# MarkJhonBao/InfantPoseEstimation_GaussianBias

Measured on AMD Instinct MI355X. Metric: images/sec (train fwd+bwd) HRFormer-S 256x192, higher is better.
Workload: dtype bf16; 1 GPU; HRFormer-small + fusion head, 256x192 -> 64x48, K=17, train step fwd+bwd+AdamW, DropPath 0.1, BN train; global_batch=64, per_gpu_batch=64, parallelism=dp1, launch=hipGraph replay, branches on concurrent HIP streams

## Files before the change

infantposeestimation_gaussianbias_amd/csrc/pk_block.hip:

```cpp
#include "pk_common.h"

typedef __attribute__((ext_vector_type(8))) short bf16x8;
typedef __attribute__((ext_vector_type(4))) float f32x4;
typedef __attribute__((ext_vector_type(4))) short s16x4;
typedef __attribute__((ext_vector_type(4))) unsigned int u32x4;
typedef __attribute__((ext_vector_type(2))) unsigned int u32x2;

#define OOB_OFF 0x80000000u
#define MAKE_RSRC(ptr) __builtin_amdgcn_make_buffer_rsrc(const_cast<uint16_t*>(ptr), 0, 0x7ffffff0, 0x00020000)
#define LOG2E_F 1.44269504088896340736f
#define MFMA(a, b, c) __builtin_amdgcn_mfma_f32_16x16x32_bf16(a, b, c, 0, 0, 0)
#define MFMA16(a, b, c) __builtin_amdgcn_mfma_f32_16x16x16bf16_1k(a, b, c, 0, 0, 0)
#define LO4(v) __builtin_shufflevector(v, v, 0, 1, 2, 3)
#define HI4(v) __builtin_shufflevector(v, v, 4, 5, 6, 7)
#define LDS_FENCE() asm volatile("s_waitcnt lgkmcnt(0)" ::: "memory")

struct MlpArgs {
    const uint16_t* x;
    const uint16_t* dy;
    uint16_t* out;
    const float *gamma, *beta, *b1, *b2;
    const float* scale;
    const uint16_t* w1;
    const uint16_t* w2;
// ... 302 lines not shown
        for (int s = 0; s < NS; ++s) {
            if (!RESIDENT) {
                __syncthreads();
                if (s + 1 < NS) write_slice((s + 1) & 1);
                if (s + 2 < NS) load_slice(s + 2);
            }
            const u32x4* fr = ring + (RESIDENT ? s : (s & 1)) * NF * 64;
            f32x4 h[RT][2];
#pragma unroll
            for (int u = 0; u < 2; ++u) {
                const f32x4 bias = *reinterpret_cast<const f32x4*>(&sB1[32 * s + 8 * g + 4 * u]);
#pragma unroll
                for (int rt = 0; rt < RT; ++rt) h[rt][u] = bias;
            }
#pragma unroll
            for (int k = 0; k < NK; ++k)
#pragma unroll
                for (int u = 0; u < 2; ++u) {
                    const bf16x8 a = LDS_FRAG(fr, u * NK + k, lane);
#pragma unroll
                    for (int rt = 0; rt < RT; ++rt) h[rt][u] = MFMA(a, vf[rt][k], h[rt][u]);
                }
            bf16x8 hf[RT];
#pragma unroll
            for (int rt = 0; rt < RT; ++rt) {
                hf[rt] = pack2(gelu_erf_poly(h[rt][0]), gelu_erf_poly(h[rt][1]));
            }
#pragma unroll
            for (int ct = 0; ct < NCT; ++ct) {
                const bf16x8 a = LDS_FRAG(fr, 2 * NK + ct, lane);
#pragma unroll
                for (int rt = 0; rt < RT; ++rt) y[rt][ct] = MFMA(a, hf[rt], y[rt][ct]);
            }
        }
#pragma unroll
        for (int rt = 0; rt < RT; ++rt)
#pragma unroll
            for (int ct = 0; ct < NCT; ++ct) {
                const unsigned off = rbase[rt] == OOB_OFF ? OOB_OFF : rbase[rt] + (16 * ct + 4 * g) * 2;
                const u32x2 xo = __builtin_amdgcn_raw_buffer_load_b64(rx, off, 0, 0);
                const f32x4 b2v = __builtin_bit_cast(f32x4, __builtin_amdgcn_raw_buffer_load_b128(rb2, (16 * ct + 4 * g) * 4, 0, 0));
                const f32x4 o = (y[rt][ct] + b2v) * sc[rt] + unpack4(xo);
                __builtin_amdgcn_raw_buffer_store_b64(pack4(o), ro, off, 0, 0);
            }
    };
    if (RESIDENT) {
        for (int grp = blockIdx.x * WAVES + wave; grp < ngroups; grp += gridDim.x * WAVES) process(grp);
    } else {
        process(blockIdx.x * WAVES + wave);
    }
}

template <int C>
__global__ void __launch_bounds__(256) k_mlp_bwd_dx(MlpArgs p) {
    constexpr int HD = 4 * C, NK = C / 32, NT = HD / 16, NS = HD / 32, NCT = C / 16, RT = 2;
    __shared__ __attribute__((aligned(16))) u32x4 sW1[NT * NK * 64];
    __shared__ __attribute__((aligned(16))) u32x4 sW2T[NT * NK * 64];
    __shared__ __attribute__((aligned(16))) u32x4 sW1T[NCT * NS * 64];
    __shared__ __attribute__((aligned(16))) float sB1[HD];
    __shared__ float sRed[4][2][C];
    const int tid = threadIdx.x, lane_ = tid & 63, wave = tid >> 6, i16 = lane_ & 15, g = lane_ >> 4;
    stage_frags(sW1, p.w1, NT * NK, C, [](int f, int i) { return hid(f / NK, i); }, [](int f) { return 32 * (f % NK); });
    stage_frags(sW2T, p.w2t, NT * NK, C, [](int f, int i) { return hid(f / NK, i); }, [](int f) { return 32 * (f % NK); });
    stage_frags(sW1T, p.w1t, NCT * NS, HD, [](int f, int i) { return 16 * (f / NS) + i; }, [](int f) { return 32 * (f % NS); });
    for (int i = tid; i < HD; i += 256) sB1[i] = p.b1[i];
    float gam[NK][8], bet[NK][8];
#pragma unroll
    for (int k = 0; k < NK; ++k)
#pragma unroll
        for (int j = 0; j < 8; ++j) {
            gam[k][j] = p.gamma[32 * k + 8 * g + j];
            bet[k][j] = p.beta[32 * k + 8 * g + j];
        }
    f32x4 gamA[NCT], dgam[NCT], dbet[NCT];
    const f32x4 zero = {0.f, 0.f, 0.f, 0.f};
#pragma unroll
    for (int ct = 0; ct < NCT; ++ct) {
        gamA[ct] = *reinterpret_cast<const f32x4*>(p.gamma + 16 * ct + 4 * g);
        dgam[ct] = dbet[ct] = zero;
    }
    __syncthreads();
    const auto rx = MAKE_RSRC(p.x);
    const auto rg = MAKE_RSRC(p.dy);
    const auto ro = MAKE_RSRC(p.out);
    const int ngroups = (p.M + 16 * RT - 1) / (16 * RT);
    const float inv_c = 1.f / (float)C;
    for (int grp = blockIdx.x * 4 + wave; grp < ngroups; grp += gridDim.x * 4) {
        const int lane = opaque_lane<true>(lane_);
        u32x4 xr[RT][NK], dyr[RT][NK];
        u32x2 xo[RT][NCT], dyo[RT][NCT];
        unsigned rbase[RT];
        float sc[RT];
#pragma unroll
        for (int rt = 0; rt < RT; ++rt) {
            const int row = grp * 16 * RT + 16 * rt + i16;
            const bool ok = row < p.M;
            rbase[rt] = ok ? (unsigned)row * (unsigned)(C * 2) : OOB_OFF;
#pragma unroll
            for (int k = 0; k < NK; ++k) {
                const unsigned off = ok ? rbase[rt] + (32 * k + 8 * g) * 2 : OOB_OFF;
                xr[rt][k] = __builtin_amdgcn_raw_buffer_load_b128(rx, off, 0, 0);
                dyr[rt][k] = __builtin_amdgcn_raw_buffer_load_b128(rg, off, 0, 0);
            }
#pragma unroll
            for (int ct = 0; ct < NCT; ++ct) {
                const unsigned off = ok ? rbase[rt] + (16 * ct + 4 * g) * 2 : OOB_OFF;
                xo[rt][ct] = __builtin_amdgcn_raw_buffer_load_b64(rx, off, 0, 0);
                dyo[rt][ct] = __builtin_amdgcn_raw_buffer_load_b64(rg, off, 0, 0);
            }
            sc[rt] = (p.scale && ok) ? p.scale[row / p.rows_per_sample] : 1.f;
        }
        bf16x8 vf[RT][NK], gf[RT][NK];
        float mean[RT], rstd[RT];
#pragma unroll
        for (int rt = 0; rt < RT; ++rt) {
            ln_row<NK>(xr[rt], gam, bet, inv_c, p.eps, vf[rt], mean[rt], rstd[rt]);
            scale_rows<NK>(dyr[rt], sc[rt], gf[rt]);
        }
        f32x4 dv[RT][NCT];
#pragma unroll
        for (int rt = 0; rt < RT; ++rt)
#pragma unroll
            for (int ct = 0; ct < NCT; ++ct) dv[rt][ct] = zero;
#pragma unroll
        for (int s = 0; s < NS; ++s) {
            f32x4 dz[RT][2];
#pragma unroll
            for (int u = 0; u < 2; ++u) {
                const int t = 2 * s + u;
                const f32x4 bias = *reinterpret_cast<const f32x4*>(&sB1[32 * s + 8 * g + 4 * u]);
                f32x4 z[RT], dh[RT];
#pragma unroll
                for (int rt = 0; rt < RT; ++rt) {
                    z[rt] = bias;
                    dh[rt] = zero;
                }
#pragma unroll
                for (int k = 0; k < NK; ++k) {
                    const bf16x8 a1 = LDS_FRAG(sW1, t * NK + k, lane), a2 = LDS_FRAG(sW2T, t * NK + k, lane);
#pragma unroll
                    for (int rt = 0; rt < RT; ++rt) {
                        z[rt] = MFMA(a1, vf[rt][k], z[rt]);
                        dh[rt] = MFMA(a2, gf[rt][k], dh[rt]);
                    }
                }
#pragma unroll
                for (int rt = 0; rt < RT; ++rt) dz[rt][u] = dh[rt] * gelu_grad(z[rt]);
            }
            bf16x8 dzf[RT];
#pragma unroll
            for (int rt = 0; rt < RT; ++rt) dzf[rt] = pack2(dz[rt][0], dz[rt][1]);
#pragma unroll
            for (int ct = 0; ct < NCT; ++ct) {
                const bf16x8 a = LDS_FRAG(sW1T, ct * NS + s, lane);
#pragma unroll
                for (int rt = 0; rt < RT; ++rt) dv[rt][ct] = MFMA(a, dzf[rt], dv[rt][ct]);
            }
        }
#pragma unroll
        for (int rt = 0; rt < RT; ++rt) {
            f32x4 xh[NCT];
            float s1 = 0.f, s2 = 0.f;
#pragma unroll
            for (int ct = 0; ct < NCT; ++ct) {
                xh[ct] = (unpack4(xo[rt][ct]) - mean[rt]) * rstd[rt];
#pragma unroll
                for (int r = 0; r < 4; ++r) {
                    const float gh = dv[rt][ct][r] * gamA[ct][r];
                    s1 += gh;
                    s2 += gh * xh[ct][r];
                }
                dgam[ct] += dv[rt][ct] * xh[ct];
                dbet[ct] += dv[rt][ct];
            }
            s1 = xor16_sum(s1);
            s1 = xor32_sum(s1);
            s2 = xor16_sum(s2);
            s2 = xor32_sum(s2);
            const float m1 = s1 * inv_c, m2 = s2 * inv_c;
#pragma unroll
            for (int ct = 0; ct < NCT; ++ct) {
                const f32x4 o = (dv[rt][ct] * gamA[ct] - m1 - xh[ct] * m2) * rstd[rt] + unpack4(dyo[rt][ct]);
                __builtin_amdgcn_raw_buffer_store_b64(pack4(o), ro, rbase[rt] == OOB_OFF ? OOB_OFF : rbase[rt] + (16 * ct + 4 * g) * 2, 0, 0);
            }
        }
    }
#pragma unroll
    for (int ct = 0; ct < NCT; ++ct)
#pragma unroll
        for (int r = 0; r < 4; ++r) {
            float a = dgam[ct][r], b = dbet[ct][r];
            a = lanes_sum<16>(a);
            b = lanes_sum<16>(b);
            if (i16 == 0) {
                sRed[wave][0][16 * ct + 4 * g + r] = a;
                sRed[wave][1][16 * ct + 4 * g + r] = b;
            }
        }
    __syncthreads();
    if (tid < 2 * C) {
        const int which = tid / C, c = tid - which * C;
        p.part[(size_t)blockIdx.x * 2 * C + tid] = ((sRed[0][which][c] + sRed[1][which][c]) + sRed[2][which][c]) + sRed[3][which][c];
    }
}

template <int C, int HS>
__global__ void __launch_bounds__(256) k_mlp_bwd_dw(MlpArgs p) {
// ... 928 lines not shown
            f32x4 xh[NCT], gamA[NCT];
            float s1 = 0.f, s2 = 0.f;
#pragma unroll
            for (int ct = 0; ct < NCT; ++ct) {
                gamA[ct] = *reinterpret_cast<const f32x4*>(&sGam[16 * ct + 4 * g]);
                xh[ct] = (unpack4(xo4[t][ct]) - mu) * rsd;
#pragma unroll
                for (int r = 0; r < 4; ++r) {
                    const float gh = du[t][ct][r] * gamA[ct][r];
                    s1 += gh;
                    s2 += gh * xh[ct][r];
                }
                if (valid) {
                    dgam[ct] += du[t][ct] * xh[ct];
                    dbet[ct] += du[t][ct];
                }
            }
            s1 = xor16_sum(s1);
            s1 = xor32_sum(s1);
            s2 = xor16_sum(s2);
            s2 = xor32_sum(s2);
            const float m1 = s1 * inv_c, m2 = s2 * inv_c;
#pragma unroll
            for (int ct = 0; ct < NCT; ++ct) {
                const f32x4 o = (du[t][ct] * gamA[ct] - m1 - xh[ct] * m2) * rsd + unpack4(dyo4[t][ct]);
                __builtin_amdgcn_raw_buffer_store_b64(pack4(o), ro, valid ? (unsigned)rw * (unsigned)(C * 2) + (16 * ct + 4 * g) * 2 : OOB_OFF, 0, 0);
            }
        }
    }
    const int i16 = lane_ & 15, g = lane_ >> 4;
#pragma unroll
    for (int ct = 0; ct < NCT; ++ct)
#pragma unroll
        for (int r = 0; r < 4; ++r) {
            float a = dgam[ct][r], b = dbet[ct][r];
            a = lanes_sum<16>(a);
            b = lanes_sum<16>(b);
            if (i16 == 0) {
                sRed[wave][0][16 * ct + 4 * g + r] = a;
                sRed[wave][1][16 * ct + 4 * g + r] = b;
            }
        }
    __syncthreads();
    for (int i = tid; i < 4 * HEADS * 169; i += 256) {
        const int wv = i / (HEADS * 169), r = i % (HEADS * 169);
        part_rpb[((size_t)blockIdx.x * 4 + wv) * HEADS * 169 + r] = sTab[wv][r / 169][r % 169];
    }
    if (tid < 2 * C) {
        const int which = tid / C, c = tid - which * C;
        part_ln[(size_t)blockIdx.x * 2 * C + tid] = ((sRed[0][which][c] + sRed[1][which][c]) + sRed[2][which][c]) + sRed[3][which][c];
    }
}

static inline int attn_blocks(int n_windows) {
    constexpr int cap = 256;
    const int need = (n_windows + 3) / 4;
    return need < cap ? (need < 1 ? 1 : need) : cap;
}
extern "C" int pk_attn_block_blocks(int n_windows) { return attn_blocks(n_windows); }
extern "C" int pk_attn_block_bwd(const void* dy, const void* x, const int32_t* rowmap, const float* gamma, const float* beta,
                                 const float* rel_table, const void* wqkv, const float* bqkv, const void* wqkv_t, const void* wproj_t,
                                 const float* row_scale, const void* o_saved, const float* lse, void* dx, void* dqkv, void* u_out,
                                 float* ln_partial, float* rpb_partial, int n_windows, int windows_per_sample, int heads, int C, float eps,
                                 void* stream) {
    PK_SUPPORTED((C == 32 || C == 64) && heads * 32 == C, "pk_attn_block_bwd: C=%d heads=%d (built for C = 32 / 64 with head_dim 32)", C, heads);
    PK_REQUIRE(dy && x && rowmap && gamma && beta && rel_table && wqkv && bqkv && wqkv_t && wproj_t && o_saved && lse && dx && dqkv && u_out &&
               ln_partial && rpb_partial && n_windows > 0, "pk_attn_block_bwd: null pointer");
    PK_REQUIRE(!row_scale || windows_per_sample > 0, "pk_attn_block_bwd: row_scale needs windows_per_sample");
    PK_REQUIRE(((((uintptr_t)x) | ((uintptr_t)dy) | ((uintptr_t)dx) | ((uintptr_t)wqkv) | ((uintptr_t)wqkv_t) | ((uintptr_t)wproj_t) |
                 ((uintptr_t)o_saved) | ((uintptr_t)dqkv) | ((uintptr_t)u_out) | ((uintptr_t)gamma)) & 15) == 0, "pk_attn_block_bwd: 16-byte alignment");
    PK_REQUIRE((int64_t)n_windows * AT_N * 3 * C < 0x3fffffffLL, "pk_attn_block_bwd: too large for 32-bit offsets");
    AttnArgs a{};
    a.x = (const uint16_t*)x; a.dy = (const uint16_t*)dy; a.out = (uint16_t*)dx; a.rowmap = rowmap; a.gamma = gamma; a.beta = beta;
    a.table = rel_table; a.bqkv = bqkv; a.scale = row_scale; a.wqkv = (const uint16_t*)wqkv; a.wqkv_t = (const uint16_t*)wqkv_t;
    a.wproj_t = (const uint16_t*)wproj_t; a.o_save = (uint16_t*)const_cast<void*>(o_saved); a.lse = const_cast<float*>(lse);
    a.dqkv = (uint16_t*)dqkv; a.u_save = (uint16_t*)u_out; a.n_windows = n_windows;
    a.windows_per_sample = windows_per_sample > 0 ? windows_per_sample : 1; a.eps = eps; a.softmax_scale = 1.f / sqrtf(32.f);
    const dim3 grid(attn_blocks(n_windows)), block(256);
    if (C == 32) hipLaunchKernelGGL(k_attn_bwd<32>, grid, block, 0, (hipStream_t)stream, a, ln_partial, rpb_partial);
    else hipLaunchKernelGGL(k_attn_bwd<64>, grid, block, 0, (hipStream_t)stream, a, ln_partial, rpb_partial);
    return pk_launch_status("pk_attn_block_bwd");
}
extern "C" int pk_attn_block_supported(int C, int heads) { return (C == 32 || C == 64) && heads * 32 == C; }
extern "C" int pk_attn_block_fwd(const void* x, const int32_t* rowmap, const float* gamma, const float* beta, const float* rel_table,
                                 const void* wqkv, const float* bqkv, const void* wproj, const float* bproj, const float* row_scale,
                                 void* y, void* o_save, float* lse, int n_windows, int windows_per_sample, int heads, int C, float eps,
                                 void* stream) {
    PK_SUPPORTED(pk_attn_block_supported(C, heads), "pk_attn_block_fwd: C=%d heads=%d (built for C = 32 / 64 with head_dim 32)", C, heads);
    PK_REQUIRE(x && rowmap && gamma && beta && rel_table && wqkv && bqkv && wproj && bproj && y && n_windows > 0, "pk_attn_block_fwd: null pointer");
    PK_REQUIRE(!row_scale || windows_per_sample > 0, "pk_attn_block_fwd: row_scale needs windows_per_sample");
    PK_REQUIRE(((((uintptr_t)x) | ((uintptr_t)y) | ((uintptr_t)wqkv) | ((uintptr_t)wproj) | ((uintptr_t)o_save) | ((uintptr_t)bproj)) & 15) == 0,
               "pk_attn_block_fwd: 16-byte alignment");
    PK_REQUIRE((int64_t)n_windows * AT_N * 3 * C < 0x3fffffffLL, "pk_attn_block_fwd: too large for 32-bit offsets");
    AttnArgs a{};
    a.x = (const uint16_t*)x; a.out = (uint16_t*)y; a.rowmap = rowmap; a.gamma = gamma; a.beta = beta; a.table = rel_table; a.bqkv = bqkv;
    a.bproj = bproj; a.scale = row_scale; a.wqkv = (const uint16_t*)wqkv; a.wproj = (const uint16_t*)wproj; a.o_save = (uint16_t*)o_save;
    a.lse = lse; a.n_windows = n_windows; a.windows_per_sample = windows_per_sample > 0 ? windows_per_sample : 1; a.eps = eps;
    a.softmax_scale = 1.f / sqrtf(32.f);
    const dim3 grid(attn_blocks(n_windows)), block(256);
    if (C == 32) hipLaunchKernelGGL(k_attn_fwd<32>, grid, block, 0, (hipStream_t)stream, a);
    else hipLaunchKernelGGL(k_attn_fwd<64>, grid, block, 0, (hipStream_t)stream, a);
    return pk_launch_status("pk_attn_block_fwd");
}

extern "C" int pk_attn_block_wide_supported(int C, int heads, int n_windows) {
    constexpr int min_win = 1024;
// ... 181 lines not shown
```

infantposeestimation_gaussianbias_amd/nnops.py:

```python
import os

import numpy as np
import torch

from . import _lib
from ._lib import call, stream_ptr

BF16, F32, I32 = torch.bfloat16, torch.float32, torch.int32
ACT_DTYPE = BF16
WS = 7


def _e(shape, dtype, dev):
    return torch.empty(shape, dtype=dtype, device=dev)


_SINK_EPOCH = [0]


def begin_grad_epoch():
    _SINK_EPOCH[0] += 1


def sink_written(param) -> bool:
# ... 856 lines not shown
        red(0, dg, nbx, C, 2 * C, base=lnp)
        red(C, db, nbx, C, 2 * C, base=lnp)
        for y in range(ns):
            o = y * nbw * SL
            red(o, dw1, nbw, HS * C, SL, out_offset=y * HS * C)
            red(o + HS * C, dw2, nbw, C * HS, SL, layout=2, T=Hd, Cin=HS, out_stride=1, out_offset=y * HS)
            red(o + 2 * HS * C, db1, nbw, HS, SL, out_offset=y * HS)
        red(2 * HS * C + HS, dbb2, nbw, C, SL)
        if all_sinks:
            _PENDING.extend(rows)
            return dx, None, None, None, None, None, None, None
        _reduce_now(rows, dev)
        return (dx, None if sg else dg, None if sb else db, None if s_w1 else dw1, None if s_b1 else db1, None if s_w2 else dw2,
                None if s_b2 else dbb2, None)


def wide_mlp_enabled(C, hidden, M=0):
    return bool(_lib.lib.pk_ln_mlp_wide_supported(C, hidden, 0 if _wide_forced() else M))


def _wide_forced():
    return os.environ.get("POSE_FUSED_WIDE_FORCE", "0") == "1"


def wide_attn_enabled(C, heads, n_windows=0):
    return bool(_lib.lib.pk_attn_block_wide_supported(C, heads, 0 if _wide_forced() else n_windows))


def attn_half_wide_forward(x, g1, b1, table, wqkv, bqkv, wproj, bproj, scale1, heads, c_real=0, attn_scale=0.0):
    wc = _wc()
    x = x.contiguous()
    B, H, W, C = x.shape
    amap, nwin = window_rowmap(B, H, W, x.device)
    y = _e((B, H, W, C), BF16, x.device)
    s1 = None if scale1 is None else scale1.float().contiguous()
    call("pk_attn_block_wide_fwd", x, amap, g1, b1, table, wc.fwd[id(wqkv)], bqkv, wc.fwd[id(wproj)], bproj, s1, y, B * nwin, nwin, heads, C,
         c_real or C, attn_scale or float(C // heads) ** -0.5, 1e-5, stream_ptr())
    return y


def mlp_half_wide_forward(x, g2, b2, w1, bias1, w2, bias2, scale2, c_real=0):
    wc = _wc()
    x = x.contiguous()
    B, H, W, C = x.shape
    s2 = None if scale2 is None else scale2.float().contiguous()
    y = _e((B, H, W, C), BF16, x.device)
    call("pk_ln_mlp_wide_fwd", x, g2, b2, wc.fwd[id(w1)], bias1, wc.fwd[id(w2)], bias2, s2, y, B * H * W, C, c_real or C, w1.shape[0], H * W, 1e-5,
         stream_ptr())
    return y


def fused_attn_enabled(C, heads, c_real=0, attn_scale=0.0, train=True):
    ok = c_real in (0, C) and not attn_scale and bool(_lib.lib.pk_attn_block_supported(C, heads))
    return ok and C in ((32,) if train else (32, 64))


def attn_half_fused_forward(x, g1, b1, table, wqkv, bqkv, wproj, bproj, scale1, heads, save=False):
    wc = _wc()
    x = x.contiguous()
    B, H, W, C = x.shape
    amap, nwin = window_rowmap(B, H, W, x.device)
    nw = B * nwin
    y = _e((B, H, W, C), BF16, x.device)
    o = _e((nw * WS * WS, C), BF16, x.device) if save else None
    lse = _e((nw * heads * WS * WS,), F32, x.device) if save else None
    s1 = None if scale1 is None else scale1.float().contiguous()
    call("pk_attn_block_fwd", x, amap, g1, b1, table, wc.fwd[id(wqkv)], bqkv, wc.fwd[id(wproj)], bproj, s1, y, o, lse, nw, nwin, heads, C,
         1e-5, stream_ptr())
    return y, o, lse, amap


class _AttnHalfFused(torch.autograd.Function):

    @staticmethod
    def forward(ctx, x, g1, b1, table, wqkv, bqkv, wproj, bproj, scale1, heads):
        ctx.params = (g1, b1, table, wqkv, bqkv, wproj, bproj)
        wc = _wc()
        x = x.contiguous()
        y, o, lse, amap = attn_half_fused_forward(x, g1, b1, table, wqkv, bqkv, wproj, bproj, scale1, heads, save=True)
        s1 = None if scale1 is None else scale1.float().contiguous()
        ctx.save_for_backward(x, g1, b1, table, bqkv, s1 if s1 is not None else x.new_empty(0), o, lse, wc.fwd[id(wqkv)], wc.dgrad[id(wqkv)],
                              wc.dgrad[id(wproj)], amap)
        ctx.meta = (heads, s1 is not None)
        return y

    @staticmethod
    def backward(ctx, dy):
        x, g1, b1, table, bqkv, s1, o, lse, wqkv_f, wqkv_t, wproj_t, amap = ctx.saved_tensors
        heads, has_s = ctx.meta
        s1 = s1 if has_s else None
        B, H, W, C = x.shape
        dev, M = dy.device, B * H * W
        nw = amap.numel() // (WS * WS)
        nwin, Mw = nw // B, nw * WS * WS
        dy = dy.contiguous()
        pg1, pb1, ptab, pwqkv, pbqkv, pwproj, pbproj = ctx.params
        (dg, sg), (db, sb) = _sink(pg1), _sink(pb1)
        no_tab = getattr(ptab, "_pk_zero_table", False)
        dtable, s_t = (None, True) if no_tab else _sink(ptab)
        nb = _lib.lib.pk_attn_block_blocks(nw)
        small_sinks = sg and sb and s_t and deferral_enabled()
        if small_sinks:
            lnp = _workspace(dg, "attn_ln", nb * 2 * C)
            rpb = _workspace(dg if no_tab else dtable, "attn_rpb_void" if no_tab else "attn_rpb", nb * 4 * heads * 169)
        else:
            lnp, rpb = _e((nb * 2 * C,), F32, dev), _e((nb * 4 * heads * 169,), F32, dev)
        dx = _e((B, H, W, C), BF16, dev)
# ... 160 lines not shown
```

Measured before the change: 4227 images/sec.

## Drop transposed W1 LDS copy; read W1^T via ds_read_tr16 from swizzled W1

The MLP backward-dx kernel now stages W1 once in LDS in a row-major layout with an XOR swizzle, and reads the transposed fragments it needs with ds_read_tr16_b64 transpose loads instead of keeping a separate pre-fragmented W1^T copy. This removes one weight staging pass and frees LDS. A waves_per_eu occupancy hint is added as well. The risk is more per-load address math and possible LDS bank conflicts if the swizzle does not line up with the transpose-read pattern.

```diff
diff --git a/infantposeestimation_gaussianbias_amd/csrc/pk_block.hip b/infantposeestimation_gaussianbias_amd/csrc/pk_block.hip
--- a/infantposeestimation_gaussianbias_amd/csrc/pk_block.hip
+++ b/infantposeestimation_gaussianbias_amd/csrc/pk_block.hip
@@ -378,17 +378,23 @@
 }
 
 template <int C>
-__global__ void __launch_bounds__(256) k_mlp_bwd_dx(MlpArgs p) {
+__device__ __forceinline__ int w1_off(int row, int col) {
+    const int swz = C == 64 ? ((row & 2) | ((row >> 1) & 4)) : ((row >> 2) & 2);
+    return row * C + ((((col >> 3) ^ swz) << 3) | (col & 7));
+}
+template <int C>
+__global__ void __launch_bounds__(256) __attribute__((amdgpu_waves_per_eu(C == 64 ? 2 : 1))) k_mlp_bwd_dx(MlpArgs p) {
     constexpr int HD = 4 * C, NK = C / 32, NT = HD / 16, NS = HD / 32, NCT = C / 16, RT = 2;
-    __shared__ __attribute__((aligned(16))) u32x4 sW1[NT * NK * 64];
+    __shared__ __attribute__((aligned(16))) uint16_t sW1[HD * C];
     __shared__ __attribute__((aligned(16))) u32x4 sW2T[NT * NK * 64];
-    __shared__ __attribute__((aligned(16))) u32x4 sW1T[NCT * NS * 64];
     __shared__ __attribute__((aligned(16))) float sB1[HD];
     __shared__ float sRed[4][2][C];
     const int tid = threadIdx.x, lane_ = tid & 63, wave = tid >> 6, i16 = lane_ & 15, g = lane_ >> 4;
-    stage_frags(sW1, p.w1, NT * NK, C, [](int f, int i) { return hid(f / NK, i); }, [](int f) { return 32 * (f % NK); });
+    for (int idx = tid; idx < HD * C / 8; idx += 256) {
+        const int row = idx / (C / 8), col = 8 * (idx % (C / 8));
+        *reinterpret_cast<u32x4*>(&sW1[w1_off<C>(row, col)]) = *reinterpret_cast<const u32x4*>(p.w1 + row * C + col);
+    }
     stage_frags(sW2T, p.w2t, NT * NK, C, [](int f, int i) { return hid(f / NK, i); }, [](int f) { return 32 * (f % NK); });
-    stage_frags(sW1T, p.w1t, NCT * NS, HD, [](int f, int i) { return 16 * (f / NS) + i; }, [](int f) { return 32 * (f % NS); });
     for (int i = tid; i < HD; i += 256) sB1[i] = p.b1[i];
     float gam[NK][8], bet[NK][8];
 #pragma unroll
@@ -412,7 +418,13 @@
     const int ngroups = (p.M + 16 * RT - 1) / (16 * RT);
     const float inv_c = 1.f / (float)C;
     for (int grp = blockIdx.x * 4 + wave; grp < ngroups; grp += gridDim.x * 4) {
-        const int lane = opaque_lane<true>(lane_);
+        const int lane = opaque_lane<true>(lane_), li = lane & 15, lg = lane >> 4;
+        const uint16_t* w1r[NK];
+        const uint16_t* w1c[NCT];
+#pragma unroll
+        for (int k = 0; k < NK; ++k) w1r[k] = sW1 + w1_off<C>(hid(0, li), 32 * k + 8 * lg);
+#pragma unroll
+        for (int ct = 0; ct < NCT; ++ct) w1c[ct] = sW1 + w1_off<C>(8 * lg + (li >> 2), 16 * ct + 4 * (li & 3));
         u32x4 xr[RT][NK], dyr[RT][NK];
         u32x2 xo[RT][NCT], dyo[RT][NCT];
         unsigned rbase[RT];
@@ -463,7 +475,8 @@
                 }
 #pragma unroll
                 for (int k = 0; k < NK; ++k) {
-                    const bf16x8 a1 = LDS_FRAG(sW1, t * NK + k, lane), a2 = LDS_FRAG(sW2T, t * NK + k, lane);
+                    const bf16x8 a1 = __builtin_bit_cast(bf16x8, *reinterpret_cast<const u32x4*>(w1r[k] + hid(t, 0) * C));
+                    const bf16x8 a2 = LDS_FRAG(sW2T, t * NK + k, lane);
 #pragma unroll
                     for (int rt = 0; rt < RT; ++rt) {
                         z[rt] = MFMA(a1, vf[rt][k], z[rt]);
@@ -478,7 +491,10 @@
             for (int rt = 0; rt < RT; ++rt) dzf[rt] = pack2(dz[rt][0], dz[rt][1]);
 #pragma unroll
             for (int ct = 0; ct < NCT; ++ct) {
-                const bf16x8 a = LDS_FRAG(sW1T, ct * NS + s, lane);
+                const uint16_t* a0 = w1c[ct] + 32 * s * C;
+                const s16x4 lo = __builtin_amdgcn_ds_read_tr16_b64_v4i16((__attribute__((address_space(3))) s16x4*)a0);
+                const s16x4 hi = __builtin_amdgcn_ds_read_tr16_b64_v4i16((__attribute__((address_space(3))) s16x4*)(a0 + 4 * C));
+                const bf16x8 a = {lo[0], lo[1], lo[2], lo[3], hi[0], hi[1], hi[2], hi[3]};
 #pragma unroll
                 for (int rt = 0; rt < RT; ++rt) dv[rt][ct] = MFMA(a, dzf[rt], dv[rt][ct]);
             }
```

Result: no change. 4251 images/sec, median of 6 (+0.6%).

## Add fused C=64 attention-block backward kernel and enable fused path for training

Applied to the files above, without the earlier changes.

Adds a specialized k_attn_bwd<64> kernel that fuses LayerNorm recompute, QKV projection, windowed-attention backward, relative-position-bias gradient folding, dQKV-to-input projection and the LayerNorm backward for the two-head C=64 branch. Weight chunks are streamed through a double-buffered LDS ring. The Python gate now lets the fused attention path run in training for C=64 as well as C=32, replacing the unfused sequence of kernels there. The kernel carries heavy register and LDS pressure (launch bounds 256,2), which may limit occupancy.

```diff
diff --git a/infantposeestimation_gaussianbias_amd/csrc/pk_block.hip b/infantposeestimation_gaussianbias_amd/csrc/pk_block.hip
--- a/infantposeestimation_gaussianbias_amd/csrc/pk_block.hip
+++ b/infantposeestimation_gaussianbias_amd/csrc/pk_block.hip
@@ -1513,6 +1513,470 @@
     }
 }
 
+template <>
+__global__ void __launch_bounds__(256, 2) k_attn_bwd<64>(AttnArgs p, float* __restrict__ part_ln, float* __restrict__ part_rpb) {
+    constexpr int C = 64, HEADS = 2, NK = 2, NCT = 4, SLOT = 12;
+    __shared__ __attribute__((aligned(16))) u32x4 sRing[2 * SLOT * 64];
+    __shared__ __attribute__((aligned(16))) float sBqkv[3 * C];
+    __shared__ __attribute__((aligned(16))) float sGam[C], sBet[C];
+    __shared__ __attribute__((aligned(16))) int sA[64];
+    __shared__ float sBias[HEADS][176];
+    __shared__ __attribute__((aligned(16))) float sLse[4][64], sDelta[4][64];
+    __shared__ float sMean[4][64], sRstd[4][64];
+    __shared__ int sRow[4][64];
+    __shared__ float sTab[4][HEADS][192];
+    constexpr int FOLD_PAD = 296;
+    __shared__ float sFoldBuf[FOLD_PAD + 4 * AT_N * AT_N + FOLD_PAD];
+    float* const sFold0 = sFoldBuf + FOLD_PAD;
+    __shared__ __attribute__((aligned(16))) float sRed[4][2][C];
+    const int tid = threadIdx.x, lane_ = tid & 63, wave = __builtin_amdgcn_readfirstlane(tid >> 6);
+    struct Staged { u32x4 a, b, c; };
+    const auto rwq = __builtin_amdgcn_make_buffer_rsrc(const_cast<uint16_t*>(p.wqkv), 0, 3 * C * C * 2, 0x00020000);
+    const auto rwt = __builtin_amdgcn_make_buffer_rsrc(const_cast<uint16_t*>(p.wqkv_t), 0, 3 * C * C * 2, 0x00020000);
+    const auto rwp = __builtin_amdgcn_make_buffer_rsrc(const_cast<uint16_t*>(p.wproj_t), 0, C * C * 2, 0x00020000);
+    auto fetch_chunk = [&](int c) -> Staged {
+        Staged r;
+        const int ln = opaque_lane<true>(lane_), s_i = ln & 15, s_col = 32 * (wave & 1) + 8 * (ln >> 4);
+        const unsigned v_tok = (unsigned)(((16 * (wave >> 1) + s_i) * C + s_col) * 2);
+        const unsigned v_hid = (unsigned)((hid(wave >> 1, s_i) * C + s_col) * 2);
+        const unsigned v_t = (unsigned)(((16 * wave + s_i) * 3 * C + 8 * (ln >> 4)) * 2);
+        const int h = c < 6 ? (c >= 3 ? 1 : 0) : c - 6, kind = c < 6 ? (c >= 3 ? c - 3 : c) : 3;
+        const unsigned hrow = (unsigned)(32 * h * C * 2);
+        if (kind == 0) {
+            r.a = __builtin_amdgcn_raw_buffer_load_b128(rwq, v_tok, hrow, 0);
+            r.b = __builtin_amdgcn_raw_buffer_load_b128(rwq, v_tok, hrow + (unsigned)(C * C * 2), 0);
+            r.c = __builtin_amdgcn_raw_buffer_load_b128(rwq, v_tok, hrow + (unsigned)(2 * C * C * 2), 0);
+        } else if (kind == 1) {
+            r.a = __builtin_amdgcn_raw_buffer_load_b128(rwp, v_tok, hrow, 0);
+            r.b = __builtin_amdgcn_raw_buffer_load_b128(rwq, v_hid, hrow + (unsigned)(C * C * 2), 0);
+            r.c = r.a;
+        } else if (kind == 2) {
+            r.a = __builtin_amdgcn_raw_buffer_load_b128(rwq, v_hid, hrow, 0);
+            r.b = __builtin_amdgcn_raw_buffer_load_b128(rwp, v_hid, hrow, 0);
+            r.c = r.a;
+        } else {
+            r.a = __builtin_amdgcn_raw_buffer_load_b128(rwt, v_t, (unsigned)(32 * h * 2), 0);
+            r.b = __builtin_amdgcn_raw_buffer_load_b128(rwt, v_t, (unsigned)(32 * (HEADS + h) * 2), 0);
+            r.c = __builtin_amdgcn_raw_buffer_load_b128(rwt, v_t, (unsigned)(32 * (2 * HEADS + h) * 2), 0);
+        }
+        return r;
+    };
+    auto write_chunk = [&](int c, const Staged& st) {
+        u32x4* const d = sRing + (((c & 1) * SLOT + wave) * 64 + opaque_lane<true>(lane_));
+        d[0] = st.a;
+        d[4 * 64] = st.b;
+        if (c % 3 == 0 || c == 7) d[8 * 64] = st.c;
+    };
+    {
+        const Staged st = fetch_chunk(0);
+        write_chunk(0, st);
+    }
+    for (int i = tid; i < 3 * C; i += 256) sBqkv[i] = p.bqkv[i];
+    for (int i = tid; i < C; i += 256) {
+        sGam[i] = p.gamma[i];
+        sBet[i] = p.beta[i];
+    }
+    if (tid < 64) sA[tid] = tid < AT_N ? rel_a7(tid) : -1;
+    for (int i = tid; i < HEADS * 169; i += 256) sBias[i / 169][i % 169] = p.table[(i % 169) * HEADS + i / 169] * LOG2E_F;
+    for (int i = tid; i < 4 * HEADS * 192; i += 256) (&sTab[0][0][0])[i] = 0.f;
+    for (int i = tid; i < 4 * 2 * C; i += 256) (&sRed[0][0][0])[i] = 0.f;
+    __syncthreads();
+    const f32x4 zero = {0.f, 0.f, 0.f, 0.f};
+    const auto rx = MAKE_RSRC(p.x);
+    const auto rg = MAKE_RSRC(p.dy);
+    const auto ro = MAKE_RSRC(p.out);
+    const auto rs = MAKE_RSRC(p.o_save);
+    const float inv_c = 1.f / (float)C, scale = p.softmax_scale, scale2 = p.softmax_scale * LOG2E_F, inv_scale = 1.f / p.softmax_scale;
+    const int per_round = gridDim.x * 4, n_rounds = (p.n_windows + per_round - 1) / per_round;
+#pragma unroll 1
+    for (int rd = 0; rd < n_rounds; ++rd) {
+        const int w = rd * per_round + blockIdx.x * 4 + wave;
+        const bool active = w < p.n_windows;
+        if (!active) {
+#pragma unroll 1
+            for (int c = 0; c < 8; ++c) {
+                __syncthreads();
+                const Staged st = fetch_chunk((c + 1) & 7);
+                write_chunk((c + 1) & 7, st);
+            }
+            continue;
+        }
+        bf16x8 uf[4][NK], gf[4][NK];
+        uint16_t* const dq_base = p.dqkv + (size_t)w * AT_N * 3 * C;
+        {
+            const int lane = opaque_lane<true>(lane_), i16 = lane & 15, g = lane >> 4;
+            int row[4];
+            u32x4 xr[4][NK], dyr[4][NK];
+#pragma unroll
+            for (int t = 0; t < 4; ++t) {
+                const int n = 16 * t + i16;
+                row[t] = n < AT_N ? p.rowmap[w * AT_N + n] : -1;
+            }
+#pragma unroll
+            for (int t = 0; t < 4; ++t)
+#pragma unroll
+                for (int k = 0; k < NK; ++k) {
+                    const unsigned off = row[t] >= 0 ? (unsigned)row[t] * (unsigned)(C * 2) + (32 * k + 8 * g) * 2 : OOB_OFF;
+                    xr[t][k] = __builtin_amdgcn_raw_buffer_load_b128(rx, off, 0, 0);
+                    dyr[t][k] = __builtin_amdgcn_raw_buffer_load_b128(rg, off, 0, 0);
+                }
+            const float sc = p.scale ? p.scale[w / p.windows_per_sample] : 1.f;
+            float gam[NK][8], bet[NK][8];
+#pragma unroll
+            for (int k = 0; k < NK; ++k) {
+                *reinterpret_cast<f32x4*>(&gam[k][0]) = *reinterpret_cast<const f32x4*>(&sGam[32 * k + 8 * g]);
+                *reinterpret_cast<f32x4*>(&gam[k][4]) = *reinterpret_cast<const f32x4*>(&sGam[32 * k + 8 * g + 4]);
+                *reinterpret_cast<f32x4*>(&bet[k][0]) = *reinterpret_cast<const f32x4*>(&sBet[32 * k + 8 * g]);
+                *reinterpret_cast<f32x4*>(&bet[k][4]) = *reinterpret_cast<const f32x4*>(&sBet[32 * k + 8 * g + 4]);
+            }
+#pragma unroll
+            for (int t = 0; t < 4; ++t) {
+                float mean_t, rstd_t;
+                ln_row<NK>(xr[t], gam, bet, inv_c, p.eps, uf[t], mean_t, rstd_t);
+                if (g == 0) {
+                    sMean[wave][16 * t + i16] = mean_t;
+                    sRstd[wave][16 * t + i16] = rstd_t;
+                    sRow[wave][16 * t + i16] = row[t];
+                }
+                scale_rows<NK>(dyr[t], sc, gf[t]);
+                if (row[t] < 0) {
+#pragma unroll
+                    for (int k = 0; k < NK; ++k) uf[t][k] = (bf16x8){0, 0, 0, 0, 0, 0, 0, 0};
+                }
+                if (16 * t + i16 < AT_N) {
+#pragma unroll
+                    for (int k = 0; k < NK; ++k)
+                        *reinterpret_cast<bf16x8*>(p.u_save + ((size_t)w * AT_N + 16 * t + i16) * C + 32 * k + 8 * g) = uf[t][k];
+                }
+            }
+        }
+#pragma unroll 1
+        for (int h = 0; h < HEADS; ++h) {
+            bf16x8 qf[4], kf[4], vf[4], dof[4];
+            u32x2 osv[4][2];
+            float lsv[4];
+            __syncthreads();
+            const Staged st_b = fetch_chunk(3 * h + 1), st_c = fetch_chunk(3 * h + 2);
+            {
+                const int lane = opaque_lane<true>(lane_), i16 = lane & 15, g = lane >> 4;
+                const u32x4* const fa = sRing + (h & 1) * (SLOT * 64);
+#pragma unroll
+                for (int t = 0; t < 4; ++t) {
+                    const int i = 16 * t + i16;
+                    const unsigned ob = i < AT_N ? (unsigned)((w * AT_N + i) * C + 32 * h + 4 * g) * 2u : OOB_OFF;
+                    osv[t][0] = __builtin_amdgcn_raw_buffer_load_b64(rs, ob, 0, 0);
+                    osv[t][1] = __builtin_amdgcn_raw_buffer_load_b64(rs, i < AT_N ? ob + 32 : OOB_OFF, 0, 0);
+                    lsv[t] = i < AT_N ? p.lse[((size_t)w * HEADS + h) * AT_N + i] : 0.f;
+                }
+#pragma unroll
+                for (int t = 0; t < 4; ++t) {
+                    f32x4 a[3][2];
+#pragma unroll
+                    for (int et = 0; et < 2; ++et) {
+#pragma unroll
+                        for (int part = 0; part < 3; ++part) a[part][et] = *reinterpret_cast<const f32x4*>(&sBqkv[part * C + 32 * h + 16 * et + 4 * g]);
+#pragma unroll
+                        for (int k = 0; k < NK; ++k)
+#pragma unroll
+                            for (int part = 0; part < 3; ++part) a[part][et] = MFMA(LDS_FRAG(fa, 4 * part + 2 * et + k, lane), uf[t][k], a[part][et]);
+                    }
+                    qf[t] = pack2(a[0][0], a[0][1]);
+                    kf[t] = pack2(a[1][0], a[1][1]);
+                    vf[t] = pack2(a[2][0], a[2][1]);
+                    __builtin_amdgcn_sched_barrier(0);
+                }
+            }
+            write_chunk(3 * h + 1, st_b);
+            __syncthreads();
+            write_chunk(3 * h + 2, st_c);
+            Staged st_n;
+            {
+                const int lane = opaque_lane<true>(lane_), i16 = lane & 15, g = lane >> 4;
+                const u32x4* const fb = sRing + ((h + 1) & 1) * (SLOT * 64);
+#pragma unroll
+                for (int t = 0; t < 4; ++t) {
+                    f32x4 a[2] = {zero, zero};
+#pragma unroll
+                    for (int et = 0; et < 2; ++et)
+#pragma unroll
+                        for (int k = 0; k < NK; ++k) a[et] = MFMA(LDS_FRAG(fb, 2 * et + k, lane), gf[t][k], a[et]);
+                    dof[t] = pack2(a[0], a[1]);
+                    const int i = 16 * t + i16;
+                    const f32x4 o0 = unpack4(osv[t][0]), o1 = unpack4(osv[t][1]);
+                    float de = 0.f;
+#pragma unroll
+                    for (int r = 0; r < 4; ++r) de += a[0][r] * o0[r] + a[1][r] * o1[r];
+                    de = xor16_sum(de);
+                    de = xor32_sum(de);
+                    if (g == 0) {
+                        sLse[wave][i] = -lsv[t] * inv_scale;
+                        sDelta[wave][i] = -de;
+                    }
+                    __builtin_amdgcn_sched_barrier(0);
+                }
+                bf16x8 Kt[2][2];
+#pragma unroll
+                for (int ce = 0; ce < 2; ++ce) {
+                    f32x4 a[4];
+                    const float bk = sBqkv[C + 32 * h + hid(ce, i16)];
+#pragma unroll
+                    for (int t = 0; t < 4; ++t) a[t] = (f32x4){bk, bk, bk, bk};
+#pragma unroll
+                    for (int k = 0; k < NK; ++k) {
+                        const bf16x8 wk = LDS_FRAG(fb, 4 + 2 * ce + k, lane);
+#pragma unroll
+                        for (int t = 0; t < 4; ++t) a[t] = MFMA(uf[t][k], wk, a[t]);
+                    }
+#pragma unroll
+                    for (int s = 0; s < 2; ++s) Kt[s][ce] = pack2(a[2 * s], a[2 * s + 1]);
+                    __builtin_amdgcn_sched_barrier(0);
+                }
+                LDS_FENCE();
+                __builtin_amdgcn_sched_barrier(0);
+#pragma unroll
+                for (int ci = 0; ci < 4; ++ci) {
+                    const int i = 16 * ci + i16;
+                    const bool iok = ci < 3 || i16 == 0;
+                    const int ai = rel_a7(iok ? i : 0) + 84;
+                    const float li = sLse[wave][i], di = sDelta[wave][i];
+                    const f32x4 li4 = {li, li, li, li}, di4 = {di, di, di, di};
+                    f32x4 dq[2] = {zero, zero};
+#pragma unroll
+                    for (int s = 0; s < 2; ++s) {
+                        f32x4 ds[2];
+#pragma unroll
+                        for (int u = 0; u < 2; ++u) {
+                            const int cj = 2 * s + u;
+                            const f32x4 scr = MFMA(kf[cj], qf[ci], li4), dp = MFMA(vf[cj], dof[ci], di4);
+                            const int4 aj = *reinterpret_cast<const int4*>(&sA[16 * cj + 4 * g]);
+                            const int ajr[4] = {aj.x, aj.y, aj.z, aj.w};
+#pragma unroll
+                            for (int r = 0; r < 4; ++r) {
+                                const bool jv = cj < 3 || (g == 0 && r == 0);
+                                const int e = ai - (cj < 3 ? ajr[r] : max(ajr[r], 0));
+                                const float ev = __builtin_amdgcn_exp2f(__builtin_fmaf(scr[r], scale2, sBias[h][e]));
+                                const float pv = (iok && jv) ? ev : 0.f;
+                                ds[u][r] = pv * dp[r];
+                                if (iok && jv) sFold0[wave * (AT_N * AT_N) + i * AT_N + 16 * cj + 4 * g + r] = ds[u][r];
+                            }
+                        }
+                        const bf16x8 df = pack2(ds[0], ds[1]);
+#pragma unroll
+                        for (int ce = 0; ce < 2; ++ce) dq[ce] = MFMA(Kt[s][ce], df, dq[ce]);
+                    }
+                    if (iok) {
+                        const u32x2 q0 = pack4(dq[0] * scale), q1 = pack4(dq[1] * scale);
+                        *reinterpret_cast<u32x4*>(dq_base + (size_t)i * 3 * C + 32 * h + 8 * g) = (u32x4){q0[0], q0[1], q1[0], q1[1]};
+                    }
+                    __builtin_amdgcn_sched_barrier(0);
+                }
+                st_n = fetch_chunk(3 * h + 3);
+                {
+                    LDS_FENCE();
+                    const int lane_f = opaque_lane<true>(lane_);
+                    for (int e = lane_f; e < 169; e += 64) {
+                        const int dy_ = e / 13 - 6, dx_ = e % 13 - 6;
+                        const int x0 = max(0, -dx_), x1 = min(7, 7 - dx_);
+                        const int base = wave * (AT_N * AT_N) + (dy_ * 7 + dx_) * AT_N;
+                        unsigned keep[7];
+#pragma unroll
+                        for (int xj = 0; xj < 7; ++xj) keep[xj] = (xj >= x0 && xj < x1) ? 0xffffffffu : 0u;
+                        float acc = 0.f;
+                        for (int yj = max(0, -dy_); yj < min(7, 7 - dy_); ++yj) {
+#pragma unroll
+                            for (int xj = 0; xj < 7; ++xj) {
+                                const float v = sFold0[base + yj * (7 * AT_N + 7) + xj * (AT_N + 1)];
+                                acc += __uint_as_float(__float_as_uint(v) & keep[xj]);
+                            }
+                        }
+                        sTab[wave][h][e] += acc;
+                    }
+                    LDS_FENCE();
+                }
+            }
+            __syncthreads();
+            write_chunk(3 * h + 3, st_n);
+            {
+                const int lane = opaque_lane<true>(lane_), i16 = lane & 15, g = lane >> 4;
+                const u32x4* const fc = sRing + (h & 1) * (SLOT * 64);
+                bf16x8 Qt[2][2], dOt[2][2];
+#pragma unroll
+                for (int ce = 0; ce < 2; ++ce) {
+                    f32x4 a[2][4];
+                    const float bq = sBqkv[32 * h + hid(ce, i16)];
+#pragma unroll
+                    for (int t = 0; t < 4; ++t) {
+                        a[0][t] = (f32x4){bq, bq, bq, bq};
+                        a[1][t] = zero;
+                    }
+#pragma unroll
+                    for (int k = 0; k < NK; ++k) {
+                        const bf16x8 wq = LDS_FRAG(fc, 2 * ce + k, lane), wp = LDS_FRAG(fc, 4 + 2 * ce + k, lane);
+#pragma unroll
+                        for (int t = 0; t < 4; ++t) {
+                            a[0][t] = MFMA(uf[t][k], wq, a[0][t]);
+                            a[1][t] = MFMA(gf[t][k], wp, a[1][t]);
+                        }
+                    }
+#pragma unroll
+                    for (int s = 0; s < 2; ++s) {
+                        Qt[s][ce] = pack2(a[0][2 * s], a[0][2 * s + 1]);
+                        dOt[s][ce] = pack2(a[1][2 * s], a[1][2 * s + 1]);
+                    }
+                }
+#pragma unroll
+                for (int cj = 0; cj < 4; ++cj) {
+                    const int j = 16 * cj + i16;
+                    const bool jok = cj < 3 || i16 == 0;
+                    const int ajn = 84 - rel_a7(jok ? j : 0);
+                    f32x4 dv[2] = {zero, zero}, dk[2] = {zero, zero};
+#pragma unroll
+                    for (int s = 0; s < 2; ++s) {
+                        f32x4 pp[2], ds[2];
+#pragma unroll
+                        for (int u = 0; u < 2; ++u) {
+                            const int ci = 2 * s + u;
+                            const f32x4 l4 = *reinterpret_cast<const f32x4*>(&sLse[wave][16 * ci + 4 * g]);
+                            const f32x4 de4 = *reinterpret_cast<const f32x4*>(&sDelta[wave][16 * ci + 4 * g]);
+                            const f32x4 scr = MFMA(qf[ci], kf[cj], l4), dp = MFMA(dof[ci], vf[cj], de4);
+                            const int4 aq = *reinterpret_cast<const int4*>(&sA[16 * ci + 4 * g]);
+                            const int aqr[4] = {aq.x, aq.y, aq.z, aq.w};
+#pragma unroll
+                            for (int r = 0; r < 4; ++r) {
+                                const bool iv = ci < 3 || (g == 0 && r == 0);
+                                const float ev = __builtin_amdgcn_exp2f(__builtin_fmaf(scr[r], scale2, sBias[h][(ci < 3 ? aqr[r] : max(aqr[r], 0)) + ajn]));
+                                const float pv = (jok && iv) ? ev : 0.f;
+                                pp[u][r] = pv;
+                                ds[u][r] = pv * dp[r];
+                            }
+                        }
+                        const bf16x8 pf = pack2(pp[0], pp[1]), df = pack2(ds[0], ds[1]);
+#pragma unroll
+                        for (int ce = 0; ce < 2; ++ce) {
+                            dv[ce] = MFMA(dOt[s][ce], pf, dv[ce]);
+                            dk[ce] = MFMA(Qt[s][ce], df, dk[ce]);
+                        }
+                    }
+                    if (jok) {
+                        const u32x2 k0 = pack4(dk[0] * scale), k1 = pack4(dk[1] * scale), v0 = pack4(dv[0]), v1 = pack4(dv[1]);
+                        *reinterpret_cast<u32x4*>(dq_base + (size_t)j * 3 * C + C + 32 * h + 8 * g) = (u32x4){k0[0], k0[1], k1[0], k1[1]};
+                        *reinterpret_cast<u32x4*>(dq_base + (size_t)j * 3 * C + 2 * C + 32 * h + 8 * g) = (u32x4){v0[0], v0[1], v1[0], v1[1]};
+                    }
+                    __builtin_amdgcn_sched_barrier(0);
+                }
+                LDS_FENCE();
+            }
+        }
+        asm volatile("s_waitcnt vmcnt(0)" ::: "memory");
+        f32x4 du[4][NCT];
+#pragma unroll
+        for (int t = 0; t < 4; ++t)
+#pragma unroll
+            for (int ct = 0; ct < NCT; ++ct) du[t][ct] = zero;
+#pragma unroll
+        for (int h = 0; h < HEADS; ++h) {
+            __syncthreads();
+            const Staged st_e = fetch_chunk((7 + h) & 7);
+            {
+                const int lane = opaque_lane<true>(lane_), i16 = lane & 15, g = lane >> 4;
+                const u32x4* const fe = sRing + (h & 1) * (SLOT * 64);
+                u32x4 dfr[4][3];
+#pragma unroll
+                for (int t = 0; t < 4; ++t)
+#pragma unroll
+                    for (int part = 0; part < 3; ++part) {
+                        dfr[t][part] = (u32x4){0u, 0u, 0u, 0u};
+                        if (t < 3 || i16 == 0)
+                            dfr[t][part] = *reinterpret_cast<const u32x4*>(dq_base + (size_t)(16 * t + i16) * 3 * C + part * C + 32 * h + 8 * g);
+                    }
+#pragma unroll
+                for (int t = 0; t < 4; ++t)
+#pragma unroll
+                    for (int part = 0; part < 3; ++part)
+#pragma unroll
+                        for (int ct = 0; ct < NCT; ++ct)
+                            du[t][ct] = MFMA(LDS_FRAG(fe, 4 * part + ct, lane), __builtin_bit_cast(bf16x8, dfr[t][part]), du[t][ct]);
+            }
+            write_chunk((7 + h) & 7, st_e);
+        }
+        {
+            const int lane = opaque_lane<true>(lane_), i16 = lane & 15, g = lane >> 4;
+            u32x2 xo4[4][NCT], dyo4[4][NCT];
+            int row2[4];
+            f32x4 dgam[NCT], dbet[NCT];
+#pragma unroll
+            for (int ct = 0; ct < NCT; ++ct) dgam[ct] = dbet[ct] = zero;
+#pragma unroll
+            for (int t = 0; t < 4; ++t) row2[t] = sRow[wave][16 * t + i16];
+            auto request = [&](int t) {
+#pragma unroll
+                for (int ct = 0; ct < NCT; ++ct) {
+                    const unsigned off = row2[t] >= 0 ? (unsigned)row2[t] * (unsigned)(C * 2) + (16 * ct + 4 * g) * 2 : OOB_OFF;
+                    xo4[t][ct] = __builtin_amdgcn_raw_buffer_load_b64(rx, off, 0, 0);
+                    dyo4[t][ct] = __builtin_amdgcn_raw_buffer_load_b64(rg, off, 0, 0);
+                }
+            };
+            request(0);
+#pragma unroll
+            for (int t = 0; t < 4; ++t) {
+                if (t + 1 < 4) request(t + 1);
+                const int rw = row2[t];
+                const float mu = sMean[wave][16 * t + i16], rsd = sRstd[wave][16 * t + i16];
+                const bool valid = rw >= 0;
+                f32x4 xh[NCT], gamA[NCT];
+                float s1 = 0.f, s2 = 0.f;
+#pragma unroll
+                for (int ct = 0; ct < NCT; ++ct) {
+                    gamA[ct] = *reinterpret_cast<const f32x4*>(&sGam[16 * ct + 4 * g]);
+                    xh[ct] = (unpack4(xo4[t][ct]) - mu) * rsd;
+#pragma unroll
+                    for (int r = 0; r < 4; ++r) {
+                        const float gh = du[t][ct][r] * gamA[ct][r];
+                        s1 += gh;
+                        s2 += gh * xh[ct][r];
+                    }
+                    if (valid) {
+                        dgam[ct] += du[t][ct] * xh[ct];
+                        dbet[ct] += du[t][ct];
+                    }
+                }
+                s1 = xor16_sum(s1);
+                s1 = xor32_sum(s1);
+                s2 = xor16_sum(s2);
+                s2 = xor32_sum(s2);
+                const float m1 = s1 * inv_c, m2 = s2 * inv_c;
+#pragma unroll
+                for (int ct = 0; ct < NCT; ++ct) {
+                    const f32x4 o = (du[t][ct] * gamA[ct] - m1 - xh[ct] * m2) * rsd + unpack4(dyo4[t][ct]);
+                    __builtin_amdgcn_raw_buffer_store_b64(pack4(o), ro, valid ? (unsigned)rw * (unsigned)(C * 2) + (16 * ct + 4 * g) * 2 : OOB_OFF, 0, 0);
+                }
+            }
+#pragma unroll
+            for (int ct = 0; ct < NCT; ++ct) {
+                f32x4 a, b;
+#pragma unroll
+                for (int r = 0; r < 4; ++r) {
+                    a[r] = lanes_sum<16>(dgam[ct][r]);
+                    b[r] = lanes_sum<16>(dbet[ct][r]);
+                }
+                if (i16 == 0) {
+                    *reinterpret_cast<f32x4*>(&sRed[wave][0][16 * ct + 4 * g]) += a;
+                    *reinterpret_cast<f32x4*>(&sRed[wave][1][16 * ct + 4 * g]) += b;
+                }
+            }
+        }
+    }
+    __syncthreads();
+    for (int i = tid; i < 4 * HEADS * 169; i += 256) {
+        const int wv = i / (HEADS * 169), r = i % (HEADS * 169);
+        part_rpb[((size_t)blockIdx.x * 4 + wv) * HEADS * 169 + r] = sTab[wv][r / 169][r % 169];
+    }
+    if (tid < 2 * C) {
+        const int which = tid / C, c = tid - which * C;
+        part_ln[(size_t)blockIdx.x * 2 * C + tid] = ((sRed[0][which][c] + sRed[1][which][c]) + sRed[2][which][c]) + sRed[3][which][c];
+    }
+}
+
 static inline int attn_blocks(int n_windows) {
     constexpr int cap = 256;
     const int need = (n_windows + 3) / 4;
diff --git a/infantposeestimation_gaussianbias_amd/nnops.py b/infantposeestimation_gaussianbias_amd/nnops.py
--- a/infantposeestimation_gaussianbias_amd/nnops.py
+++ b/infantposeestimation_gaussianbias_amd/nnops.py
@@ -932,7 +932,7 @@
 
 def fused_attn_enabled(C, heads, c_real=0, attn_scale=0.0, train=True):
     ok = c_real in (0, C) and not attn_scale and bool(_lib.lib.pk_attn_block_supported(C, heads))
-    return ok and C in ((32,) if train else (32, 64))
+    return ok and C in (32, 64)
 
 
 def attn_half_fused_forward(x, g1, b1, table, wqkv, bqkv, wproj, bproj, scale1, heads, save=False):
```

Result: faster. 4214 images/sec before, 4261 images/sec after, median of 6 (+1.1%).
